# Rorisis/Co-Occ

Hardware: AMD Instinct MI355X
Metric: samples/sec (6-cam frame + sweep -> occ+render), 200x200x16 grid (higher is better)
Workload: dtype f32 (split-f16 products, fp32 accumulate)

## Files before the change

co_occ_amd/_lib.py:

```python
import ctypes
import os
import threading
import time

import torch

_HERE = os.path.dirname(os.path.abspath(__file__))
LIB_PATH = os.path.join(_HERE, "libcoocc_hip.so")

c_int, c_float, c_void_p, c_size_t, c_int64 = (ctypes.c_int, ctypes.c_float, ctypes.c_void_p,
                                               ctypes.c_size_t, ctypes.c_int64)


class ConvDesc(ctypes.Structure):
    _fields_ = [(n, c_void_p) for n in ("in_", "w", "out", "scale", "bias", "res", "gather", "out_rows", "ws")] + \
               [("ws_floats", c_int64)] + \
               [(n, c_int) for n in ("M", "Cin", "Cout", "taps", "in_stride", "out_stride", "res_stride",
                                     "B", "Xi", "Yi", "Zi", "Xo", "Yo", "Zo", "ksize", "stride", "pad",
                                     "relu", "res_mode", "splitk", "tile_hint", "kx", "ky", "kz", "px", "py", "pz",
                                     "wgroup_rows", "mfma_dtype")] + [("alpha", ctypes.c_float), ("M_dev", c_void_p), ("gather_stride", c_int), ("out16", c_void_p), ("out16_stride", c_int), ("out_h2", c_int),
                                                                   ("out_h2_twin", c_void_p), ("tile_sem", c_void_p), ("tile_sem_ints", c_int),
                                                                  ("alpha_dev", c_void_p), ("sx", c_int), ("sy", c_int), ("sz", c_int)]


# ... 40 lines not shown
    "coocc_ball_query": (I, [I, I, I, F, F, I, P, P, P, P]),
    "coocc_knn_topk": (I, [I, I, I, P, P, P, P, P]),
    "coocc_voxel_index_map": (I, [P, I, I, P, P]),
    "coocc_voxel_index_map_dev": (I, [P, I, P, I, P, P]),
    "coocc_fine_sample_voxel_dev": (I, [P, I, I, I, I, P, I, P, I, P, P, P, I, P]),
    "coocc_fine_sample_img_dev": (I, [P, I, I, I, I, P, P, L, P, P, I, I, P]),
    "coocc_fine_mlp_pre_dev": (I, [P, I, P, I, L, P, I, P, P, P, F, P, P, P, P, F, P, P, I, P, P]),
    "coocc_fine_fused": (I, [P, I, I, I, P, I, I, I, P, P, I, P, I, P, P, P, P, F, P, P, P, P, F, P, P, I, P, P, P]),
    "coocc_fine2_pack": (I, [P, P, I, P, P, P, P, P, P, P, P, P, P]),
    "coocc_fine2_h2": (I, [P, I, I, I, I, P, I, I, I, P, P, I, P, P, P, P, F, F, I, P, P, P, P]),
    "coocc_fine_sample_img_lin": (I, [P, I, I, I, I, P, P, I, I, I, P, P, I, I, P]),
    "coocc_scatter_fine_dev": (I, [P, L, P, I, I, I, P, P, I, I, I, F, P]),
    "coocc_scatter_fine_grouped": (I, [P, I, I, P, I, P, I, I, I, I, P, F, P, P]),
    "coocc_ball_query_voxels": (I, [I, F, F, I, I, I, I, P, P, P, P, P]),
    "coocc_knn_topk_voxels": (I, [I, I, I, I, I, I, P, P, P, P, I, P, P, P, P, P]),
    "coocc_knn_assign": (I, [I, I, I, I, F, P, P, P, P, P, P]),
    "coocc_knn_threshold": (I, [I, F, P, P, P, P]),
    "coocc_index_rows_i32": (I, [P, I, P, I, P, P]),
    "coocc_conv_pack_weights": (L, [P, I, I, I, I, P]),
    "coocc_conv_fwd": (I, [ctypes.POINTER(ConvDesc), P]),
    "coocc_fuser_search_ws": (Z, [ctypes.POINTER(SearchDesc)]),
    "coocc_fuser_search": (I, [ctypes.POINTER(SearchDesc), P, P]),
    "coocc_upsample_add_trilinear": (I, [P, P, I, I, I, I, I, I, I, I, P]),
    "coocc_upsample_add_trilinear_ex": (I, [P, P, I, I, I, I, I, I, I, I, P, P]),
    "coocc_occhead_mix": (I, [P, P, I, P, P, I, I, P]),
    "coocc_occhead_mix_ex": (I, [P, P, I, P, P, I, I, P, P]),
    "coocc_argmax_flags": (I, [P, I, I, I, I, P, P]),
    "coocc_fine_sample_voxel": (I, [P, I, I, I, I, P, I, I, P, P, P, I, P]),
    "coocc_fine_sample_img": (I, [P, I, I, I, I, P, P, L, P, I, I, P]),
    "coocc_fine_mlp_pre": (I, [P, I, P, I, L, P, P, P, F, P, P, P, P, F, P, P, I, P, P]),
    "coocc_fine_mlp": (I, [P, I, P, I, L, P, P, P, P, F, P, P, P, P, F, P, P, I, P, P]),
    "coocc_groupnorm_rows": (I, [P, L, I, I, I, P, P, F, I, P]),
    "coocc_groupnorm_nhwc": (I, [P, I, I, I, I, P, P, F, I, P]),
    "coocc_scatter_fine": (I, [P, L, I, I, P, P, I, I, I, F, P]),
    "coocc_camera_mats": (I, [P, P, P, P, P, P, I, I, I, I, P, P]),
    "coocc_get_geometry": (I, [P, P, P, P, I, I, I, I, P, P]),
    "coocc_bev_pool_forward": (I, [P, P, P, P, I, I, I, I, I, I, I, P, P]),
    "coocc_bev_pool_backward": (I, [P, P, P, P, I, I, I, I, I, I, I, P, P]),
    "coocc_voxel_pool_ws": (Z, [I, I]),
    "coocc_voxel_pool": (I, [P, P, I, I, I, P, I, I, I, I, P, I, P, Z, I, P]),
    "coocc_lift_splat": (I, [P, P, P, I, I, I, I, I, I, P, I, I, I, I, P, I, P, Z, I, P]),
    "coocc_lift_splat_cams": (I, [P, P, P, P, P, P, I, I, I, I, I, I, P, I, I, I, I, P, I, P, Z, I, P]),
    "coocc_lift_splat_reuse": (I, [P, P, I, I, I, I, I, I, I, I, I, P, I, P, Z, P]),
    "coocc_bev_pool_coords": (I, [P, P, I, I, I, I, I, I, P, I, P, Z, I, P]),
    "coocc_render_nearest": (I, [P, I, I, I, P, P, I, I, I, I, P, I, P, P]),
    "coocc_render_nearest_cams": (I, [P, I, I, I, P, P, P, P, P, I, I, I, I, P, I, P, P]),
    "coocc_render_activate_table": (I, [P, I, P]),
    "coocc_upsample_maps": (I, [P, I, I, I, I, P, P, P]),
    "coocc_volume_sampling": (I, [P, I, I, I, I, P, I, P, P, P, P]),
    "coocc_raw2outputs": (I, [P, P, I, I, I, F, F, P, P, P, P]),
    "coocc_render_losses": (I, [P, P, P, P, L, I, P, P, Z, P]),
    "coocc_conv_pack_weights_dev": (L, [P, I, I, I, I, P, P]),
    "coocc_wino_pack_weights_dev": (L, [P, I, I, I, I, P, P]),
    "coocc_wino_pack_weights_h2_dev": (L, [P, I, I, I, I, P, P]),
    "coocc_conv_pack_weights_h2_dev": (L, [P, I, I, I, I, P, P]),
    "coocc_wino_gradout": (I, [P, I, I, I, I, I, I, I, P, L, P]),
    "coocc_wino_ztap_table": (I, [L, I, P, P]),
    "coocc_wino_wgrad": (I, [P, P, L, I, I, I, I, P, P, I, P, L, P]),
    "coocc_rows_to_kh2": (I, [P, I, L, L, I, F, P, P, P]),
    "coocc_wino_operand_kh2": (I, [I, P, I, I, I, I, I, I, I, P, L, F, P, P]),
    "coocc_conv_wgrad_h2": (I, [P, P, L, I, I, F, P, P, I, P, L, P]),
    "coocc_wino_wgrad_h2": (I, [P, P, L, I, I, I, I, F, P, P, I, P, L, P]),
    "coocc_conv_tap_table": (I, [I, I, I, I, I, I, I, I, I, I, I, P, P]),
    "coocc_conv_epilogue_bwd": (I, [P, I, P, I, P, I, I, I, P, I, P, I, I, P, I, P, L, P]),
    "coocc_conv_epilogue_bwd_ex": (I, [P, I, P, I, P, I, I, I, P, I, P, I, I, P, I, P, L, P, P, F, P]),
    "coocc_conv_wgrad": (I, [P, I, I, P, I, P, I, I, I, I, P, I, P, L, P]),
    "coocc_conv_wgrad_h2t": (I, [P, I, I, P, I, P, I, I, I, I, P, P, I, P, L, P]),
    "coocc_gather_rows": (I, [P, I, P, I, I, P, I, P]),
    "coocc_scatter_add_rows": (I, [P, I, P, I, I, P, I, P]),
    "coocc_voxel_pool_bwd": (I, [P, I, P, I, I, I, P, I, I, I, I, P, P]),
    "coocc_lift_splat_bwd": (I, [P, I, P, P, P, I, I, I, I, I, I, P, I, I, I, I, P, P, P]),
    "coocc_render_nearest_bwd": (I, [P, I, I, I, P, P, I, I, I, I, P, P, P, P]),
    "coocc_upsample_maps_bwd": (I, [P, P, I, I, I, I, P, P]),
    "coocc_render_losses_bwd": (I, [P, P, P, P, L, I, P, P, P, P, P]),
    "coocc_upsample_trilinear_bwd": (I, [P, P, I, I, I, I, I, I, I, I, I, P]),
    "coocc_wino_input": (I, [P, I, I, I, I, I, I, I, P, L, P]),
    "coocc_wino_input_strided": (I, [P, I, I, I, I, I, I, I, P, I, L, P]),
    "coocc_sparse_tap_sum": (I, [P, P, I, I, I, I, I, P, P, I, I, P]),
    "coocc_wino_output": (I, [P, L, I, I, I, I, I, I, P, I, P, P, P, I, I, P]),
    "coocc_wino_output_ex": (I, [P, L, I, I, I, I, I, I, P, I, P, P, P, I, I, P, P]),
    "coocc_h2_overflow": (I, [I]),
    "coocc_device_fault": (I, [I]),
    "coocc_render_heads_h2": (I, [P, I, I, I, P, P, P, P, P, P, I, P, P, P, I, P]),
    "coocc_projection_params": (I, [P, P, P, P, P, P, I, P, P, P]),
    "coocc_occhead_mix_bwd": (I, [P, P, I, P, P, P, P, I, I, P]),
    "coocc_fine_sample_voxel_bwd": (I, [P, I, I, I, I, I, P, L, P, P, P]),
    "coocc_groupnorm_rows_bwd": (I, [P, P, P, L, I, I, I, P, F, I, P, P, P, P]),
    "coocc_fine_sample_img_bwd": (I, [P, I, I, I, I, I, P, P, L, P, P]),
    "coocc_groupnorm_nhwc_bwd": (I, [P, P, P, I, I, I, I, P, F, I, P, P, P, P]),
    "coocc_voxelize_ws": (Z, [I]),
    "coocc_voxelize_hard": (I, [P, I, I, P, P, I, I, P, P, P, P, P, Z, P]),
    "coocc_vfe_mean": (I, [P, P, I, I, I, I, P, I, P]),
    "coocc_sparse_index_map": (I, [P, I, I, I, I, P, P]),
    "coocc_sparse_conv_table": (I, [P, I, I, I, I, I, I, I, P, P, P]),
    "coocc_sparse_down_flags": (I, [P, I, I, I, I, I, I, I, P, P]),
    "coocc_sparse_conv_table3": (I, [P, I, I, I, I, I, I, I, I, I, I, I, I, I, P, P, P]),
    "coocc_sparse_down_flags3": (I, [P, I, I, I, I, I, I, I, I, I, I, I, I, I, I, I, I, P, P]),
    "coocc_sparse_lin_to_coors": (I, [P, I, I, I, I, P, P, P]),
    "coocc_bn_stats": (I, [P, I, I, I, P, P, P, Z, P]),
    "coocc_bn_apply": (I, [P, I, I, P, P, P, P, F, P, I, P, P]),
    "coocc_bn_backward": (I, [P, P, P, I, I, P, P, P, F, I, P, P, P, P, P, Z, P]),
    "coocc_bn_backward_sums": (I, [P, P, P, I, I, P, P, F, I, P, P, P, Z, P]),
    "coocc_bn_backward_dx": (I, [P, P, P, I, I, P, P, P, F, I, P, P, ctypes.c_double, P, P, P]),
    "coocc_predict_labels": (I, [P, L, L, L, L, I, I, I, I, I, I, I, P, P]),
    "coocc_eval_semantic": (I, [P, L, L, L, L, I, I, I, I, P, P, I, I, I, I, I, P, P]),
    "coocc_fpn_sum": (I, [P, P, I, I, I, I, I, I, P, I, P, P]),
    "coocc_zyx_to_rows": (I, [P, P, I, I, I, I, I, I, I, P]),
    "coocc_conv_tap_table3": (I, [I] * 17 + [P, P]),
    "coocc_fpn_sum_bwd": (I, [P, I, P, P, I, I, I, I, I, I, P]),
    "coocc_lidarseg_points": (I, [P, L, L, L, L, I, I, I, I, P, L, L, I, I, P, I, I, P, P, I, P, P]),
    "coocc_render_eval_stats": (L, [P, P, P, P, I, I, I, P, P, Z, P]),
    "coocc_render_panels": (I, [P, P, P, P, I, I, I, P, P]),
    "coocc_render_eval_ssim": (L, [P, P, I, I, I, ctypes.c_double, P, P, Z, P]),
    "coocc_sparse_dgrad_table3": (I, [P] + [I] * 16 + [P, P, P, P]),
    "coocc_bn_apply_ex": (I, [P, I, I, P, P, P, P, F, P, I, P, P, P]),
    "coocc_pool_labels": (I, [P, I, I, I, I, I, I, I, P, P]),
    "coocc_occ_loss_ws": (Z, [L, I]),
    "coocc_occ_loss_fwd": (I, [P, L, I, I, P, P, I, I, I, P, P, I, P, P, P, P, Z, P]),
    "coocc_occ_loss_bwd": (I, [P, L, I, I, P, P, I, P, P, P, P, I, P]),
    "coocc_depth_labels": (I, [P, I, I, I, I, F, F, I, P, P, P]),
    "coocc_depth_bce_ws": (Z, [L, I]),
    "coocc_depth_bce": (I, [P, P, I, I, I, I, F, P, P, P, Z, P]),
    "coocc_depth_bce_bwd": (I, [P, P, I, I, I, I, F, P, P, P, P]),
    "coocc_nbr_table2d": (I, [I, I, I, I, P, P]),
    "coocc_dcn_cols": (I, [P, I, P, I, I, I, I, I, I, I, I, P, P]),
    "coocc_se_gate2": (I, [P, I, I, I, I, P, P, P, P, P]),
    "coocc_cam_mean_ws": (Z, [I, I, I]),
    "coocc_cam_mean": (I, [P, I, I, I, I, P, P, Z, P]),
    "coocc_cam_bias_relu": (I, [P, I, I, I, I, P, I, P]),
    "coocc_dcn_cols_bwd": (I, [P, I, P, I, I, I, I, I, I, I, I, P, P, P, P]),
    "coocc_se_gate2_bwd_ws": (Z, [I, I, I]),
    "coocc_se_gate2_bwd": (I, [P, I, I, I, I, P, P, P, P, P, P, P, P, Z, P]),
    "coocc_cam_sum": (I, [P, I, I, I, I, P, P, Z, P]),
    "coocc_cam_add": (I, [P, P, I, I, I, P, F, P]),
    "coocc_dropout_rows": (I, [P, P, L, I, F, P, P]),
    "coocc_img_stem": (I, [P, I, I, I, P, P, P, I, I, I, P, I, P, P]),
    "coocc_maxpool2d_rows": (I, [P, I, I, I, I, I, P, I, P, P]),
    "coocc_maxpool2d_rows_bwd": (I, [P, I, P, I, I, I, I, I, P, I, P]),
    "coocc_img_stem_wgrad_ws": (Z, [I, I, I]),
    "coocc_img_stem_wgrad": (I, [P, I, I, I, P, I, I, P, P, Z, P]),
    "coocc_optim_chunk": (I, []),
    "coocc_optim_sumsq": (I, [P, P, I, P, I, P, P]),
    "coocc_optim_clip_coef": (I, [P, I, F, P, P, P, P]),
    "coocc_optim_adamw": (I, [P, P, I, P, I, P, I, P]),
    "coocc_optim_scale": (I, [P, P, I, P, I, P, P]),
    "coocc_frames_to_imgs": (I, [P, P, I, I, I, P, P, P, L, I, I, P, P, P]),
    "coocc_points_to_depth_maps": (I, [P, L, I, P, I, I, I, P, P]),
}

_lib = None


class KernelTimer:

    def __init__(self):
        self.enabled = False
        self.only = None
        self.records = []

    class _Region:
        def __init__(self, owner, tag, work):
            self.o, self.tag, self.work = owner, tag, work

        def __enter__(self):
            lvl = int(self.o.enabled)
            self.on = lvl >= 2 or (lvl == 1 and self.work > 0 and (self.o.only is None or self.tag.startswith(self.o.only)))
# ... 162 lines not shown
```

co_occ_amd/head.py:

```python
import collections
import threading

import numpy as np
import torch
from torch import nn

from . import _lib
from . import core as core_mod
from ._lib import TIMER, call, host_f32, host_i32, ptr
from .backbone import build_bn
from .core import PackCache, PackedConv, Rows, conv_rows, linear_rows, to_rows
from .registry import HEADS

_I32, _F32, _I64 = torch.int32, torch.float32, torch.int64
_FINE_LOCK = threading.Lock()
FUSED_FINE_MLP = __import__("os").environ.get("COOCC_FUSED_FINE_MLP", "1") != "0"
FINE_LINEAR_FIRST = __import__("os").environ.get("COOCC_FINE_LINEAR_FIRST", "1") != "0"
FINE_FUSED = int(__import__("os").environ.get("COOCC_FINE_FUSED", "1"))
FINE2_H2 = __import__("os").environ.get("COOCC_FINE2_H2", "1") != "0"
FINE2_IMG_INSIDE = __import__("os").environ.get("COOCC_FINE2_IMG_INSIDE", "1") == "1"
MERGED_PRED_Q = __import__("os").environ.get("COOCC_MERGED_PRED_Q", "1") != "0"
SCATTER_GROUPED = __import__("os").environ.get("COOCC_SCATTER_GROUPED", "1") != "0"


def _conv3d(conv_cfg, cin, cout, k, pad):
    cfg = dict(conv_cfg or dict(type='Conv3d'))
    t = cfg.pop("type", "Conv3d")
    if t != "Conv3d":
        raise NotImplementedError("OccHead: conv type %r" % t)
    return nn.Conv3d(cin, cout, kernel_size=k, stride=1, padding=pad, **cfg)


@HEADS.register_module()
class OccHead(nn.Module):
    def __init__(self, in_channels, out_channel, num_level=1, num_img_level=1, soft_weights=False,
                 loss_weight_cfg=None, conv_cfg=dict(type='Conv3d', bias=False),
                 norm_cfg=dict(type='GN', num_groups=32, requires_grad=True), fine_topk=20000,
                 point_cloud_range=[-51.2, -51.2, -5.0, 51.2, 51.2, 3.0], final_occ_size=[256, 256, 20],
                 empty_idx=0, visible_loss=False, balance_cls_weight=True, cascade_ratio=1,
                 sample_from_voxel=False, sample_from_img=False, train_cfg=None, test_cfg=None,
                 padding_mode='border', data_type='nus'):
        super().__init__()
        if type(in_channels) is not list:
            in_channels = [in_channels]
        if data_type != 'nus':
            raise NotImplementedError("OccHead: only the nuScenes projection branch is implemented")
        self.in_channels, self.out_channel, self.num_level = in_channels, out_channel, num_level
        self.fine_topk = fine_topk
        self.point_cloud_range = torch.tensor(np.array(point_cloud_range)).float()
        self.final_occ_size = final_occ_size
        self.cascade_ratio = cascade_ratio
        self.sample_from_voxel, self.sample_from_img = sample_from_voxel, sample_from_img
        self.padding_mode, self.data_type = padding_mode, data_type
        self.empty_idx, self.soft_weights = empty_idx, soft_weights
        self.num_img_level, self.num_point_sampling_feat = num_img_level, num_level
        lw = loss_weight_cfg or {}
        self.loss_weight_cfg = loss_weight_cfg
        self.loss_voxel_ce_weight = lw.get('loss_voxel_ce_weight', 1.0)
        self.loss_voxel_sem_scal_weight = lw.get('loss_voxel_sem_scal_weight', 1.0)
        self.loss_voxel_geo_scal_weight = lw.get('loss_voxel_geo_scal_weight', 1.0)
        self.loss_voxel_lovasz_weight = lw.get('loss_voxel_lovasz_weight', 1.0)
        from .losses import nusc_class_weights
        self.class_weights = nusc_class_weights() if balance_cls_weight else torch.ones(17) / 17
        self.visible_loss = visible_loss
        self.device_losses = False

        if cascade_ratio != 1 and (sample_from_voxel or sample_from_img):
            fine_in = 128 if sample_from_voxel else 0
            if sample_from_img:
                self.img_mlp_0 = nn.Sequential(nn.Conv2d(512, 128, 1, 1, 0), nn.GroupNorm(16, 128), nn.ReLU(inplace=True))
                self.img_mlp = nn.Sequential(nn.Linear(128, 64), nn.GroupNorm(16, 64), nn.ReLU(inplace=True))
                fine_in += 64
            self.fine_mlp = nn.Sequential(nn.Linear(fine_in, 64), nn.GroupNorm(16, 64), nn.ReLU(inplace=True),
                                          nn.Linear(64, out_channel))
        self.occ_convs = nn.ModuleList()
        for i in range(num_level):
            mid = in_channels[i] // 2
            self.occ_convs.append(nn.Sequential(_conv3d(conv_cfg, in_channels[i], mid, 3, 1), build_bn(norm_cfg, mid),
                                                nn.ReLU(inplace=True)))
        self.occ_pred_conv = nn.Sequential(_conv3d(conv_cfg, mid, mid // 2, 1, 0), build_bn(norm_cfg, mid // 2),
                                           nn.ReLU(inplace=True), _conv3d(conv_cfg, mid // 2, out_channel, 1, 0))
        if soft_weights:
            self.voxel_soft_weights = nn.Sequential(_conv3d(conv_cfg, mid, mid // 2, 1, 0), build_bn(norm_cfg, mid // 2),
                                                    nn.ReLU(inplace=True), _conv3d(conv_cfg, mid // 2, num_level, 1, 0))
        self._packs = PackCache(self)

    def _packed(self):
        def seq2(m):
            return (PackedConv(m[0].weight, bn=m[1], bias=m[0].bias, ksize=1),
                    PackedConv(m[3].weight, bias=m[3].bias, ksize=1))

        def build():
            d = dict(occ=[PackedConv(m[0].weight, bn=m[1], bias=m[0].bias, ksize=3, pad=1) for m in self.occ_convs],
                     pred=seq2(self.occ_pred_conv))
            if self.soft_weights:
                d["soft"] = seq2(self.voxel_soft_weights)
            if hasattr(self, "fine_mlp"):
                d["fine0"] = PackedConv(self.fine_mlp[0].weight, bias=self.fine_mlp[0].bias)
                d["fine3"] = PackedConv(self.fine_mlp[3].weight, bias=self.fine_mlp[3].bias)
            if hasattr(self, "img_mlp"):
                d["img0"] = PackedConv(self.img_mlp_0[0].weight.flatten(1), bias=self.img_mlp_0[0].bias)
                d["img"] = PackedConv(self.img_mlp[0].weight, bias=self.img_mlp[0].bias)
                if self.sample_from_voxel and self.fine_mlp[0].weight.shape[1] == 192:
                    d["img_nb"] = PackedConv(self.img_mlp[0].weight)
                    d["f0_vox_nb"] = PackedConv(self.fine_mlp[0].weight[:, :128].contiguous())
                    m = self.occ_pred_conv
                    if m[0].weight.shape[0] == 64 and m[0].weight.shape[1] == 128:
                        from .core import fold_bn
                        pq = PackedConv(torch.cat([m[0].weight.flatten(1), self.fine_mlp[0].weight[:, :128]], 0).contiguous())
                        sc, bi = fold_bn(m[1], m[0].bias)
                        dev = m[0].weight.device
                        pq.scale = torch.cat([sc.float().cpu(), torch.ones(64)]).to(dev).contiguous()
                        pq.bias = torch.cat([bi.float().cpu(), torch.zeros(64)]).to(dev).contiguous()
                        pq.ksize, pq.pad = 1, 0
                        d["pred_q"] = pq
            if hasattr(self, "img_mlp") and hasattr(self, "fine_mlp"):
                d["mlp_aligned"] = all(q.data_ptr() % 16 == 0 for m in (self.img_mlp, self.fine_mlp) for q in m.parameters())
                if ("img_nb" in d and self.out_channel <= 32 and self.img_mlp[1].num_groups == 16 and self.fine_mlp[1].num_groups == 16
                        and self.fine_mlp[0].weight.is_cuda):
                    dev = self.fine_mlp[0].weight.device
                    wp = torch.empty(24576, device=dev, dtype=torch.uint8)
                    cn = torch.empty(416, device=dev, dtype=_F32)
                    li, gi, l0, g0, l3 = self.img_mlp[0], self.img_mlp[1], self.fine_mlp[0], self.fine_mlp[1], self.fine_mlp[3]
                    q = lambda t: ptr(t.detach().float().contiguous())
                    call("coocc_fine2_pack", q(l0.weight), q(l3.weight), self.out_channel, q(li.bias), q(gi.weight), q(gi.bias),
                         q(l0.bias), q(g0.weight), q(g0.bias), q(l3.bias), ptr(wp), ptr(cn))
                    d["fine2"] = (wp, cn)
            return d
        return self._packs.get_modules((self,), build)

    def forward_coarse_rows(self, voxel_feats):
        from . import core
        p = self._packed()
        feats = [to_rows(f) for f in voxel_feats]
        lbr = core.Fork(2, feats[0].t.device, enable=len(feats) > 1 and not self.training)
        with lbr:
            small = [conv_rows(f, p["occ"][i], relu=True) for i, f in enumerate(feats) if i > 0]
        o0 = conv_rows(feats[0], p["occ"][0], relu=True, twin_for=((p["soft"][0],) if self.soft_weights else ()))
        occs = [o0] + small
        wlogit = None
        if self.soft_weights:
            h = conv_rows(o0, p["soft"][0], relu=True)
            wlogit = conv_rows(h, p["soft"][1], relu=False).t
        lbr.join(*[o.t for o in small])
        L = len(occs)
        levels = (_lib.c_void_p * L)(*[o.t.data_ptr() for o in occs])
        dims = host_i32([v for o in occs for v in (o.X, o.Y, o.Z)])
        out = Rows(torch.empty_like(o0.t), o0.B, o0.X, o0.Y, o0.Z, o0.C)
        tw = None
        merged = (MERGED_PRED_Q and "pred_q" in p and core.CONV_DTYPE == "f32" and self.cascade_ratio == 2 and self._fine2_h2_ok()
                  and not self.training)
        first = p["pred_q"] if merged else p["pred"][0]
        if core.wants_h2_twin(out, (first,)):
            tw = out.h2 = torch.empty_like(o0.t)
        call("coocc_occhead_mix_ex", levels, dims, L, ptr(wlogit), ptr(out.t), o0.B, o0.C, ptr(tw))
        if merged:
            hq = conv_rows(out, first, relu=64)
            h = Rows(hq.t, hq.B, hq.X, hq.Y, hq.Z, 64, 0)
            out.aux = dict(q=hq.t[:, 64:])
        else:
            h = conv_rows(out, p["pred"][0], relu=True)
        occ = conv_rows(h, p["pred"][1], relu=False)
        return out, occ

    def level_readers(self):
        return [(pc,) for pc in self._packed()["occ"]]

    def forward_coarse_voxel(self, voxel_feats):
        out, occ = self.forward_coarse_rows(voxel_feats)
        return {'out_voxel_feats': [out.as_ncdhw()], 'occ': [occ.as_ncdhw()]}

    def _image_rows(self, p, img_feats, transform, grid_rows, dev):
        f = img_feats[0]
        _, N_i, C_i, Hf, Wf = f.shape
        rows = torch.empty(N_i * Hf * Wf, C_i, device=dev, dtype=_F32)
        call("coocc_ncdhw_to_ndhwc", ptr(f[0].float().contiguous()), ptr(rows), N_i, C_i, Hf * Wf, C_i, 0)
        g = linear_rows(rows, p["img0"])
        gn = self.img_mlp_0[1]
        call("coocc_groupnorm_nhwc", ptr(g), N_i, Hf * Wf, g.shape[1], gn.num_groups, ptr(gn.weight.detach()),
             ptr(gn.bias.detach()), float(gn.eps), 1)
        params = self._projection_params(transform, grid_rows, dev)
        return g, params, (N_i, Hf, Wf)

    def fork_image_branch(self, img_feats, transform, grid_rows):
        if not (self.sample_from_img and img_feats is not None and self.cascade_ratio != 1 and not self.training and core_mod.BRANCHES):
            return None
        dev = img_feats[0].device
        br = core_mod.Fork(1, dev)
        if not br.on:
            return None
        with br:
            out = self._image_rows(self._packed(), img_feats, transform, grid_rows, dev)
        return br, out, (grid_rows.X, grid_rows.Y, grid_rows.Z)

    def _fine(self, ovf, occ, img_feats, transform, static=False, image_branch=None):
        p = self._packed()
        dev = ovf.t.device
        V, r = ovf.V, self.cascade_ratio
        assert ovf.B == 1, "OccHead fine branch: B == 1 (as the render block asserts, coocc_ray.py:571)"
        flags = torch.empty(V, device=dev, dtype=torch.uint8)
        call("coocc_argmax_flags", ptr(occ.t), V, occ.C, occ.stride, self.empty_idx, ptr(flags))
        lin = torch.empty(V, device=dev, dtype=_I32)
        cnt = torch.empty(1, device=dev, dtype=_I32)
        ws = torch.empty(V // 1024 + 2, device=dev, dtype=_I32)
        fgmap = torch.empty(V, device=dev, dtype=_I32) if SCATTER_GROUPED else None
        call("coocc_compact_flags_ex", ptr(flags), V, ptr(lin), ptr(cnt), ptr(fgmap), ptr(ws), ws.numel() * 4)
        use_img = self.sample_from_img and img_feats is not None
        if use_img and image_branch is not None:
            br, (g, params, (N_i, Hf, Wf)), grid = image_branch
            br.join(g, params)
            if grid != (ovf.X, ovf.Y, ovf.Z):
                params = self._projection_params(transform, ovf, dev)
        elif use_img:
            g, params, (N_i, Hf, Wf) = self._image_rows(p, img_feats, transform, ovf, dev)
        if static:
            return self._fine_static(p, ovf, lin, cnt, g if use_img else None, params if use_img else None, (N_i, Hf, Wf) if use_img else None,
                                     fgmap=fgmap)
        n = int(_lib.host_read(cnt)[0])
        core_mod.check_h2_overflow()
        assert n > 0, 'no foreground in coarse voxel'
        nf = n * r ** 3
        fine_xyz = torch.empty(3, nf, device=dev, dtype=_I64)
        self._note_fine(dict(xyz=fine_xyz, lin=lin, n=n, cnt=None, coarse=(ovf.X, ovf.Y, ovf.Z), map=fgmap))
        cvox = 128 if self.sample_from_voxel else 0
        fused = (FUSED_FINE_MLP and use_img and self.sample_from_voxel and ovf.C == 128 and g.shape[1] == 128
                 and self.out_channel <= 32 and self.img_mlp[1].num_groups == 16 and self.fine_mlp[1].num_groups == 16
                 and p.get("mlp_aligned", False))
        if fused and FINE_LINEAR_FIRST and "img_nb" in p:
            P = linear_rows(g, p["img_nb"])
            fused_one = self._fused_fine_ok(ovf, N_i)
            Q = ovf.aux.get("q") if (fused_one and ovf.aux and self._fine2_h2_ok() and FINE_FUSED < 2) else None
            if Q is None:
                Q = linear_rows(ovf.t, p["f0_vox_nb"], in_coff=ovf.coff, in_C=128)
            if fused_one:
                logits = torch.empty(nf, self.out_channel, device=dev, dtype=_F32)
                self._fine_fused(p, ovf, Q, P, params, (N_i, Hf, Wf), lin, n, None, fine_xyz, logits)
                return logits, fine_xyz
            vq = torch.empty(nf, 64, device=dev, dtype=_F32)
            call("coocc_fine_sample_voxel", ptr(Q), 64, ovf.X, ovf.Y, ovf.Z, ptr(lin), n, r,
                 host_i32(self.final_occ_size), ptr(fine_xyz), ptr(vq), 64)
            samp = torch.empty(nf, 64, device=dev, dtype=_F32)
            call("coocc_fine_sample_img", ptr(P), N_i, 64, Hf, Wf, ptr(params), ptr(fine_xyz), nf, ptr(samp), 64, r if r in (2, 4) else 0)
            li, gi, l0, g0, l3 = self.img_mlp[0], self.img_mlp[1], self.fine_mlp[0], self.fine_mlp[1], self.fine_mlp[3]
            logits = torch.empty(nf, self.out_channel, device=dev, dtype=_F32)
            d = lambda t: ptr(t.detach())
            with TIMER.region("k_fine_mlp<pre>", 2.0 * nf * 64 * (64 + self.out_channel)):
                call("coocc_fine_mlp_pre", ptr(samp), 64, ptr(vq), 64, nf, d(li.bias), d(gi.weight), d(gi.bias), float(gi.eps),
                     d(l0.weight), d(l0.bias), d(g0.weight), d(g0.bias), float(g0.eps), d(l3.weight), d(l3.bias),
                     self.out_channel, ptr(logits))
            return logits, fine_xyz
        cat = torch.empty(nf, cvox if fused else cvox + (64 if use_img else 0), device=dev, dtype=_F32)
        vox_feat = cat if self.sample_from_voxel else torch.empty(nf, ovf.C, device=dev, dtype=_F32)
        call("coocc_fine_sample_voxel", ptr(ovf.t), ovf.C, ovf.X, ovf.Y, ovf.Z, ptr(lin), n, r,
             host_i32(self.final_occ_size), ptr(fine_xyz), ptr(vox_feat), vox_feat.shape[1])
        if use_img:
            samp = torch.empty(nf, g.shape[1], device=dev, dtype=_F32)
            call("coocc_fine_sample_img", ptr(g), N_i, g.shape[1], Hf, Wf, ptr(params), ptr(fine_xyz), nf, ptr(samp),
                 samp.shape[1], r if r in (2, 4) else 0)
            if fused:
                li, gi, l0, g0, l3 = self.img_mlp[0], self.img_mlp[1], self.fine_mlp[0], self.fine_mlp[1], self.fine_mlp[3]
                logits = torch.empty(nf, self.out_channel, device=dev, dtype=_F32)
                d = lambda t: ptr(t.detach())
                with TIMER.region("k_fine_mlp", 2.0 * nf * 64 * (128 + 192 + self.out_channel)):
                    call("coocc_fine_mlp", ptr(samp), samp.shape[1], ptr(cat), cat.shape[1], nf,
                         d(li.weight), d(li.bias), d(gi.weight), d(gi.bias), float(gi.eps),
                         d(l0.weight), d(l0.bias), d(g0.weight), d(g0.bias), float(g0.eps),
                         d(l3.weight), d(l3.bias), self.out_channel, ptr(logits))
                return logits, fine_xyz
            linear_rows(samp, p["img"], out=cat, out_coff=cvox)
            gn = self.img_mlp[1]
            sub = cat[:, cvox:]
            call("coocc_groupnorm_rows", _lib.c_void_p(sub.data_ptr()), nf, 64, cat.shape[1], gn.num_groups,
                 ptr(gn.weight.detach()), ptr(gn.bias.detach()), float(gn.eps), 1)
        h = linear_rows(cat, p["fine0"])
        gn = self.fine_mlp[1]
        call("coocc_groupnorm_rows", ptr(h), nf, h.shape[1], h.shape[1], gn.num_groups, ptr(gn.weight.detach()),
             ptr(gn.bias.detach()), float(gn.eps), 1)
        return linear_rows(h, p["fine3"]), fine_xyz

    def _fine_static(self, p, ovf, lin, cnt, g, params, img_dims, fgmap=None):
        dev = ovf.t.device
        V, r = ovf.V, self.cascade_ratio
        ok = (FUSED_FINE_MLP and FINE_LINEAR_FIRST and g is not None and self.sample_from_voxel and ovf.C == 128 and g.shape[1] == 128
              and self.out_channel <= 32 and self.img_mlp[1].num_groups == 16 and self.fine_mlp[1].num_groups == 16
# ... 244 lines not shown
```

include/coocc_hip.h:

```cpp
#ifndef COOCC_HIP_H
#define COOCC_HIP_H

#include <stddef.h>
#include <stdint.h>

#ifdef __cplusplus
extern "C" {
#endif

#define COOCC_OK 0
#define COOCC_EINVAL (-1)
#define COOCC_EHIP (-2)
#define COOCC_ENOMEM (-3)

const char* coocc_last_error(void);
int coocc_abi_version(void);

int coocc_device_cu_count(int* n);
int coocc_stream_create_cu_mask(const uint32_t* mask_host, int nwords, void** stream_out);
int coocc_stream_destroy(void* stream);

int coocc_event_create(int flags, void** event_out);
int coocc_event_destroy(void* event);
int coocc_event_record(void* event, void* stream);
// ... 66 lines not shown
                          const int32_t* map_k, const uint32_t* offsets, int noff, const float* q, const float* key,
                          float* val, int32_t* idx, void* stream);

int coocc_knn_topk(int nq, int nk, int K, const float* q, const float* key, float* val,
                   int32_t* idx, void* stream);

int coocc_knn_assign(int nc, int K, int ns, int nq, float dist_thresh, const float* val,
                     const int32_t* nn, const int32_t* group, int32_t* winner, int32_t* out,
                     void* stream);
int coocc_knn_threshold(int nq, float dist_thresh, const float* val, const int32_t* nn,
                        int32_t* out, void* stream);
int coocc_index_rows_i32(const int32_t* base, int nbase, const int32_t* sel, int n, int32_t* rows,
                         void* stream);


int64_t coocc_conv_pack_weights(const float* w_host, int Cout, int Cin, int taps, int tap_major,
                                float* packed_host);

typedef struct coocc_conv_desc {
  const float* in;
  const float* w;
  float* out;
  const float* scale;
  const float* bias;
  const float* res;
  const int32_t* gather;
  const int32_t* out_rows;
  float* ws;
  int64_t ws_floats;
  int M, Cin, Cout, taps;
  int in_stride, out_stride, res_stride;
  int B, Xi, Yi, Zi, Xo, Yo, Zo, ksize, stride, pad;
  int relu, res_mode;
  int splitk;
  int tile_hint;
  int kx, ky, kz;
  int px, py, pz;
  int wgroup_rows;
  int mfma_dtype;
  float alpha;
  const int32_t* M_dev;
  int gather_stride;
  void* out16;
  int out16_stride;
  int out_h2;
  void* out_h2_twin;
  int32_t* tile_sem;
  int tile_sem_ints;
  const float* alpha_dev;
  int sx, sy, sz;
} coocc_conv_desc;

int coocc_conv_fwd(const coocc_conv_desc* d, void* stream);

int coocc_rows_to_bf16(const float* in, int in_stride, int64_t rows, int C, void* out_bf16, void* stream);

int coocc_rows_to_h2(const float* in, int in_stride, int64_t rows, int C, float scale, void* out_h2, void* stream);
int coocc_rows_to_h2_ex(const float* in, int in_stride, int64_t rows, int C, float scale, const float* scale_dev, void* out_h2,
                        void* stream);
int coocc_rows_to_f16(const float* in, int in_stride, int64_t rows, int C, void* out_f16, void* stream);
int coocc_rows_to_h2_gather(const float* in, int in_stride, const int32_t* row_ids, int64_t n_cap, const int32_t* n_dev,
                            int C, float scale, void* out_h2, void* stream);

int coocc_wino_input(const float* in, int in_stride, int B, int X, int Y, int Z, int C, int tile, float* V,
                     int64_t group_rows, void* stream);
int coocc_wino_input_strided(const float* in, int in_stride, int B, int X, int Y, int Z, int C, int tile, float* V,
                             int vstride, int64_t group_rows, void* stream);
int coocc_wino_input_h2(const float* in, int in_stride, int B, int X, int Y, int Z, int C, int tile, void* V,
                        int vstride, int64_t group_rows, float scale, void* stream);
int coocc_wino_input_h2_ex(const float* in, int in_stride, int B, int X, int Y, int Z, int C, int tile, void* V,
                           int vstride, int64_t group_rows, float scale, const float* scale_dev, void* stream);
int coocc_sparse_tap_sum(const float* P, const int32_t* map, int B, int X, int Y, int Z, int Cout, const float* scale,
                         float* S, int s_stride, int p_rows, void* stream);
int coocc_wino_output(const float* Mb, int64_t group_rows, int B, int X, int Y, int Z, int C, int tile, float* out,
                      int out_stride, const float* scale, const float* bias, const float* res, int res_stride,
                      int relu, void* stream);
int coocc_wino_output_ex(const float* Mb, int64_t group_rows, int B, int X, int Y, int Z, int C, int tile, float* out,
                         int out_stride, const float* scale, const float* bias, const float* res, int res_stride,
                         int relu, void* out_h2_twin, void* stream);
int coocc_render_heads_h2(const void* x_h2, int V, int Cin, int width, const void* ws0_pack, const float* bs0,
                          const float* ws1, const float* bs1, const void* const* wr_packs_host,
                          const float* const* br_host, int n_rgb_hidden, const float* wr_out, const float* br_out,
                          float* table, int activate, void* stream);
int64_t coocc_wino_pack_weights_h2_dev(const float* w, int Cout, int Cin, int tile, int dgrad, void* packed, void* stream);
int64_t coocc_conv_pack_weights_h2_dev(const float* w, int Cout, int Cin, int taps, int mode, void* packed, void* stream);
int coocc_h2_overflow(int reset);
#define COOCC_FAULT_SPARSE_ORDINAL 1
int coocc_device_fault(int reset);
int64_t coocc_wino_pack_weights_dev(const float* w, int Cout, int Cin, int tile, int dgrad, float* packed, void* stream);
int coocc_wino_gradout(const float* dy, int dy_stride, int B, int X, int Y, int Z, int C, int tile, float* dM,
                       int64_t group_rows, void* stream);
int coocc_wino_ztap_table(int64_t rows_total, int Z, int32_t* table, void* stream);
int coocc_wino_wgrad(const float* V, const float* dM, int64_t group_rows, int Z, int Cin, int Cout, int tile,
                     const int32_t* ztap_table, float* dw, int accumulate, float* ws, int64_t ws_floats,
                     void* stream);
int coocc_rows_to_kh2(const float* x, int stride, int64_t rows, int64_t rows_pad, int C, float scale, const float* scale_dev,
                      void* out_kh2, void* stream);
int coocc_wino_operand_kh2(int which, const float* x, int x_stride, int B, int X, int Y, int Z, int C, int tile, void* out_kh2,
                           int64_t group_rows, float scale, const float* scale_dev, void* stream);
int coocc_conv_wgrad_h2(const void* x_kh2, const void* dy_kh2, int64_t rows_pad, int Cin, int Cout, float alpha,
                        const float* alpha_dev, float* dw, int accumulate, float* ws, int64_t ws_floats, void* stream);
int coocc_wino_wgrad_h2(const void* V_kh2, const void* dM_kh2, int64_t group_rows, int Z, int Cin, int Cout, int tile,
                        float alpha, const float* alpha_dev, float* dw, int accumulate, float* ws, int64_t ws_floats,
                        void* stream);

int64_t coocc_conv_pack_weights_dev(const float* w, int Cout, int Cin, int taps, int mode, float* packed,
                                    void* stream);
int coocc_conv_tap_table(int B, int Xi, int Yi, int Zi, int Xo, int Yo, int Zo, int ksize, int stride, int pad,
                         int dgrad, int32_t* table, void* stream);
int coocc_conv_epilogue_bwd(const float* dout, int dout_stride, const float* out, int out_stride,
                            const float* scale, int M, int C, int relu, float* dacc, int dacc_stride,
                            float* dres, int dres_stride, int dres_accumulate, float* dbias,
                            int dbias_accumulate, float* ws, int64_t ws_floats, void* stream);
#define COOCC_AMAX_WORDS 2048
int coocc_conv_epilogue_bwd_ex(const float* dout, int dout_stride, const float* out, int out_stride,
                               const float* scale, int M, int C, int relu, float* dacc, int dacc_stride,
                               float* dres, int dres_stride, int dres_accumulate, float* dbias,
                               int dbias_accumulate, float* ws, int64_t ws_floats, uint32_t* amax_word, float* scale2,
                               float target, void* stream);
int coocc_conv_wgrad(const float* in, int in_rows, int in_stride, const float* dacc, int dacc_stride,
                     const int32_t* table, int M, int Cin, int Cout, int taps, float* dw, int accumulate,
                     float* ws, int64_t ws_floats, void* stream);
int coocc_conv_wgrad_h2t(const float* in, int in_rows, int in_stride, const float* dacc, int dacc_stride,
                         const int32_t* table, int M, int Cin, int Cout, int taps, const float* scale2,
                         float* dw, int accumulate, float* ws, int64_t ws_floats, void* stream);

int coocc_gather_rows(const float* src, int src_stride, const int32_t* idx, int n, int C, float* dst,
                      int dst_stride, void* stream);
int coocc_scatter_add_rows(const float* src, int src_stride, const int32_t* idx, int n, int C, float* dst,
                           int dst_stride, void* stream);
int coocc_voxel_pool_bwd(const float* dout, int dout_stride, const float* geom, int npts, int pts_per_batch,
                         int C, const float* lo_dx_host, int B, int X, int Y, int Z, float* dx, void* stream);
int coocc_lift_splat_bwd(const float* dout, int dout_stride, const float* depth, const float* feat_nhwc,
                         const float* geom, int N, int D, int H, int W, int C, int pts_per_batch,
                         const float* lo_dx_host, int B, int X, int Y, int Z, float* d_depth,
                         float* d_feat_nhwc, void* stream);
int coocc_render_nearest_bwd(const float* table, int X, int Y, int Z, const float* geom, const float* zvals,
                             int N, int D, int H, int W, const float* bounds_host, const float* dmaps,
                             float* dtable, void* stream);
int coocc_upsample_maps_bwd(const float* drgbs, const float* ddepths, int N, int H, int W, int scale,
                            float* dmaps, void* stream);
int coocc_render_losses_bwd(const float* rgbs, const float* depths, const float* rgb_gt, const float* depth_gt,
                            int64_t npix, int D, const float* losses_out, const float* gl, float* drgbs,
                            float* ddepths, void* stream);

int coocc_upsample_trilinear_bwd(const float* dfine, float* dcoarse, int B, int C, int Xc, int Yc, int Zc, int Xf,
                                 int Yf, int Zf, int accumulate, void* stream);

int coocc_occhead_mix_bwd(const float* const* levels_host, const int* dims_host, int L, const float* wlogit,
                          const float* dout, float* const* glevels_host, float* dwlogit, int B, int C,
                          void* stream);

int coocc_fine_sample_voxel_bwd(const float* dfeat, int dfeat_stride, int C, int X, int Y, int Z,
                                const int64_t* fine_xyz, int64_t nfine, const int* final_size_host, float* dvol,
                                void* stream);
int coocc_groupnorm_rows_bwd(const float* x, const float* y, const float* dy, int64_t n, int C, int stride, int groups,
                             const float* gamma, float eps, int relu, float* dx, float* dgamma, float* dbeta,
                             void* stream);

int coocc_fine_sample_img_bwd(const float* dfeat, int dfeat_stride, int ncam, int Ci, int Hf, int Wf,
                              const float* params, const int64_t* fine_xyz, int64_t nfine, float* dimg,
                              void* stream);
int coocc_groupnorm_nhwc_bwd(const float* x, const float* y, const float* dy, int N, int HW, int C, int groups,
                             const float* gamma, float eps, int relu, float* dx, float* dgamma, float* dbeta,
                             void* stream);

// ... 269 lines not shown
```

Before: 259.8.

## Fuse occ head pointwise tail MLPs and argmax flags into single H2 kernels

Adds two HIP kernels that run the two-layer pointwise MLP tails of the occupancy head, the soft-weight branch and the prediction branch, in one launch each. The hidden activations stay in LDS instead of going through global memory between two conv_rows calls. The prediction kernel also computes the argmax non-empty flags, so the later argmax_flags launch is skipped. This cuts launches and intermediate traffic, but it depends on strict shape and route preconditions, and the second-layer hidden values are re-split to f16 pairs inside the kernel.

```diff
diff --git a/co_occ_amd/_lib.py b/co_occ_amd/_lib.py
--- a/co_occ_amd/_lib.py
+++ b/co_occ_amd/_lib.py
@@ -146,6 +146,8 @@
     "coocc_h2_overflow": (I, [I]),
     "coocc_device_fault": (I, [I]),
     "coocc_render_heads_h2": (I, [P, I, I, I, P, P, P, P, P, P, I, P, P, P, I, P]),
+    "coocc_head_pred_h2": (I, [P, I, I, P, P, P, P, P, I, I, P, P, I, P, I, I, P, P]),
+    "coocc_head_soft_h2": (I, [P, I, I, P, P, P, P, P, I, P, P, I, P, I, P]),
     "coocc_projection_params": (I, [P, P, P, P, P, P, I, P, P, P]),
     "coocc_occhead_mix_bwd": (I, [P, P, I, P, P, P, P, I, I, P]),
     "coocc_fine_sample_voxel_bwd": (I, [P, I, I, I, I, I, P, L, P, P, P]),
diff --git a/co_occ_amd/csrc/head_tail_h2.hip b/co_occ_amd/csrc/head_tail_h2.hip
--- /dev/null
+++ b/co_occ_amd/csrc/head_tail_h2.hip
@@ -0,0 +1,321 @@
+#include <string.h>
+
+#include "conv_k.h"
+#include "h2_rows.h"
+
+typedef float f32x16 __attribute__((ext_vector_type(16)));
+typedef _Float16 f16x8 __attribute__((ext_vector_type(8)));
+
+#define HT_BM 128
+#define HT_STAGE (HT_BM * 128)
+#define HT_LST 33
+#define HT_HST 68
+#define HT_SOFT_OUT 36864
+
+struct HeadTailK {
+  const char* x; long long rowbytes;
+  int M; const int32_t* M_dev;
+  const char* w1; const float* scale1; const float* bias1;
+  float* hq; int hq_stride; int write_hidden;
+  const char* w2; const float* bias2; int nout;
+  float* out; int out_stride;
+  int empty_idx; uint8_t* flags;
+  float alpha;
+  int* h2_flag;
+  const char* zrow;
+};
+
+__device__ __forceinline__ void ht_glds16(const void* g, void* l) {
+  __builtin_amdgcn_global_load_lds((const __attribute__((address_space(1))) void*)g, (__attribute__((address_space(3))) void*)l, 16, 0, 0);
+}
+
+__device__ __forceinline__ void ht_stage_tile(const HeadTailK& p, char* As, int m0, int wave, int lane) {
+  const int srow = lane >> 3, slot = lane & 7;
+  const unsigned aq = (unsigned)((slot ^ ((4 * (wave & 1) + (srow >> 1)) & 7)) * 16);
+#pragma unroll
+  for (int c = 0; c < 4; ++c)
+#pragma unroll
+    for (int j = 0; j < 4; ++j) {
+      const int m = m0 + (j * 4 + wave) * 8 + srow;
+      const char* src = m < p.M ? p.x + ((long long)m * p.rowbytes + c * 128 + aq) : p.zrow;
+      ht_glds16(src, &As[c * HT_STAGE + (j * 4 + wave) * 8 * 128]);
+    }
+}
+
+template <int TM>
+__device__ __forceinline__ void ht_layer1(const HeadTailK& p, const char* As, int ctile, int rb0, int lane, const unsigned (&fragoff)[4],
+                                          f32x16 (&hh)[TM], f32x16 (&xx)[TM]) {
+  f16x8 breg[4][2][2];
+  const char* wcur = p.w1 + (long long)ctile * 4096 + lane * 16;
+#pragma unroll
+  for (int c = 0; c < 4; ++c)
+#pragma unroll
+    for (int s2 = 0; s2 < 2; ++s2)
+#pragma unroll
+      for (int pl = 0; pl < 2; ++pl) breg[c][s2][pl] = *(const f16x8*)(wcur + c * 16384 + (s2 * 2 + pl) * 1024);
+#pragma unroll
+  for (int i = 0; i < TM; ++i)
+#pragma unroll
+    for (int r = 0; r < 16; ++r) { hh[i][r] = 0.f; xx[i][r] = 0.f; }
+  __syncthreads();
+#pragma unroll
+  for (int c = 0; c < 4; ++c) {
+#pragma unroll
+    for (int s2 = 0; s2 < 2; ++s2) {
+      f16x8 fhi[TM], flo[TM];
+#pragma unroll
+      for (int i = 0; i < TM; ++i) {
+        fhi[i] = *(const f16x8*)&As[fragoff[2 * s2 + 0] + (c * HT_STAGE + (rb0 + i) * 4096)];
+        flo[i] = *(const f16x8*)&As[fragoff[2 * s2 + 1] + (c * HT_STAGE + (rb0 + i) * 4096)];
+      }
+#pragma unroll
+      for (int i = 0; i < TM; ++i) hh[i] = __builtin_amdgcn_mfma_f32_32x32x16_f16(breg[c][s2][0], fhi[i], hh[i], 0, 0, 0);
+#pragma unroll
+      for (int i = 0; i < TM; ++i) xx[i] = __builtin_amdgcn_mfma_f32_32x32x16_f16(breg[c][s2][1], fhi[i], xx[i], 0, 0, 0);
+#pragma unroll
+      for (int i = 0; i < TM; ++i) xx[i] = __builtin_amdgcn_mfma_f32_32x32x16_f16(breg[c][s2][0], flo[i], xx[i], 0, 0, 0);
+      __builtin_amdgcn_sched_barrier(0);
+    }
+  }
+  __syncthreads();
+}
+
+__device__ __forceinline__ f32x4 ht_epi1(const HeadTailK& p, const f32x16& hh, const f32x16& xx, int j, int n, float alpha, float lo, bool relu) {
+  f32x4 v;
+#pragma unroll
+  for (int e = 0; e < 4; ++e) v[e] = hh[4 * j + e] * alpha + xx[4 * j + e] * lo;
+  if (p.scale1) v = v * *(const f32x4*)(p.scale1 + n);
+  if (p.bias1) v = v + *(const f32x4*)(p.bias1 + n);
+  if (relu) { v[0] = fmaxf(v[0], 0.f); v[1] = fmaxf(v[1], 0.f); v[2] = fmaxf(v[2], 0.f); v[3] = fmaxf(v[3], 0.f); }
+  return v;
+}
+
+__device__ __forceinline__ void ht_store_tile(const HeadTailK& p, const float* Ls, int m0, int nrows, int tid) {
+  const int nout = p.nout;
+  for (int idx = tid; idx < nrows * nout; idx += 256) {
+    const int r = idx / nout, c = idx - r * nout;
+    p.out[(size_t)(m0 + r) * p.out_stride + c] = Ls[r * HT_LST + c];
+  }
+}
+
+__global__ __launch_bounds__(256, 2) void k_head_pred_h2(HeadTailK p) {
+  constexpr int TM = 4;
+  __shared__ __attribute__((aligned(16))) char As[4 * HT_STAGE];
+  const int m0 = blockIdx.x * HT_BM;
+  if (p.M_dev) {
+    p.M = min(p.M, *p.M_dev);
+    if (m0 >= p.M) return;
+  }
+  const int tid = threadIdx.x;
+  const int wave = __builtin_amdgcn_readfirstlane(tid >> 6), lane = tid & 63;
+  const int li = lane & 31, h = lane >> 5;
+  ht_stage_tile(p, As, m0, wave, lane);
+  unsigned fragoff[4];
+#pragma unroll
+  for (int q = 0; q < 4; ++q) {
+    const int sl = (q & 1) * 4 + 2 * (q >> 1) + h;
+    fragoff[q] = li * 128 + ((sl ^ ((li >> 1) & 7)) << 4);
+  }
+  const float alpha = p.alpha, lo = alpha * (1.f / H2_LO_SCALE);
+  const unsigned swz = (unsigned)((li >> 1) & 7);
+  {
+    f32x16 hh[TM], xx[TM];
+    ht_layer1<TM>(p, As, wave, 0, lane, fragoff, hh, xx);
+    const int nb = wave * 32 + 4 * h;
+    const bool hidden = wave < 2;
+#pragma unroll
+    for (int i = 0; i < TM; ++i) {
+      const int m = m0 + i * 32 + li;
+#pragma unroll
+      for (int j = 0; j < 4; ++j) {
+        const int n = nb + 8 * j;
+        const f32x4 v = ht_epi1(p, hh[i], xx[i], j, n, alpha, lo, hidden);
+        if (hidden) {
+          f16x4 vh, vl;
+#pragma unroll
+          for (int e = 0; e < 4; ++e) {
+            _Float16 a, b;
+            split_h2(v[e], a, b);
+            vh[e] = a; vl[e] = b;
+          }
+          const unsigned base = (unsigned)wave * HT_STAGE + (unsigned)(i * 32 + li) * 128 + 8 * h;
+          *(f16x4*)&As[base + (((unsigned)j ^ swz) << 4)] = vh;
+          *(f16x4*)&As[base + (((unsigned)(4 + j) ^ swz) << 4)] = vl;
+          if (m < p.M) h2_guard(p.h2_flag, v);
+        }
+        if (m < p.M && (!hidden || p.write_hidden)) *(f32x4*)(p.hq + (size_t)m * p.hq_stride + n) = v;
+      }
+    }
+  }
+  f16x8 b2[2][2][2];
+  {
+    const char* wcur = p.w2 + lane * 16;
+#pragma unroll
+    for (int c = 0; c < 2; ++c)
+#pragma unroll
+      for (int s2 = 0; s2 < 2; ++s2)
+#pragma unroll
+        for (int pl = 0; pl < 2; ++pl) b2[c][s2][pl] = *(const f16x8*)(wcur + c * 16384 + (s2 * 2 + pl) * 1024);
+  }
+  f32x16 hh2, xx2;
+#pragma unroll
+  for (int r = 0; r < 16; ++r) { hh2[r] = 0.f; xx2[r] = 0.f; }
+  __syncthreads();
+#pragma unroll
+  for (int c = 0; c < 2; ++c)
+#pragma unroll
+    for (int s2 = 0; s2 < 2; ++s2) {
+      const f16x8 fhi = *(const f16x8*)&As[fragoff[2 * s2 + 0] + (c * HT_STAGE + wave * 4096)];
+      const f16x8 flo = *(const f16x8*)&As[fragoff[2 * s2 + 1] + (c * HT_STAGE + wave * 4096)];
+      hh2 = __builtin_amdgcn_mfma_f32_32x32x16_f16(b2[c][s2][0], fhi, hh2, 0, 0, 0);
+      xx2 = __builtin_amdgcn_mfma_f32_32x32x16_f16(b2[c][s2][1], fhi, xx2, 0, 0, 0);
+      xx2 = __builtin_amdgcn_mfma_f32_32x32x16_f16(b2[c][s2][0], flo, xx2, 0, 0, 0);
+    }
+  float* Ls = (float*)&As[2 * HT_STAGE];
+#pragma unroll
+  for (int j = 0; j < 4; ++j)
+#pragma unroll
+    for (int e = 0; e < 4; ++e) {
+      const int n = 8 * j + 4 * h + e;
+      float v = hh2[4 * j + e] * alpha + xx2[4 * j + e] * lo;
+      if (n < p.nout) {
+        if (p.bias2) v += p.bias2[n];
+        Ls[(wave * 32 + li) * HT_LST + n] = v;
+      }
+    }
+  __syncthreads();
+  const int nrows = min(HT_BM, p.M - m0);
+  ht_store_tile(p, Ls, m0, nrows, tid);
+  if (p.flags && tid < nrows) {
+    const float* r = Ls + tid * HT_LST;
+    float best = r[0];
+    int bi = 0;
+    for (int c = 1; c < p.nout; ++c)
+      if (r[c] > best) { best = r[c]; bi = c; }
+    p.flags[m0 + tid] = bi != p.empty_idx;
+  }
+}
+
+__global__ __launch_bounds__(256, 2) void k_head_soft_h2(HeadTailK p) {
+  constexpr int TM = 2;
+  __shared__ __attribute__((aligned(16))) char As[4 * HT_STAGE];
+  const int m0 = blockIdx.x * HT_BM;
+  if (p.M_dev) {
+    p.M = min(p.M, *p.M_dev);
+    if (m0 >= p.M) return;
+  }
+  const int tid = threadIdx.x;
+  const int wave = __builtin_amdgcn_readfirstlane(tid >> 6), lane = tid & 63;
+  const int li = lane & 31, h = lane >> 5;
+  ht_stage_tile(p, As, m0, wave, lane);
+  unsigned fragoff[4];
+#pragma unroll
+  for (int q = 0; q < 4; ++q) {
+    const int sl = (q & 1) * 4 + 2 * (q >> 1) + h;
+    fragoff[q] = li * 128 + ((sl ^ ((li >> 1) & 7)) << 4);
+  }
+  float* Hs = (float*)As;
+  {
+    const int ctile = wave & 1, rb0 = 2 * (wave >> 1);
+    const float alpha = p.alpha, lo = alpha * (1.f / H2_LO_SCALE);
+    f32x16 hh[TM], xx[TM];
+    ht_layer1<TM>(p, As, ctile, rb0, lane, fragoff, hh, xx);
+    const int nb = ctile * 32 + 4 * h;
+#pragma unroll
+    for (int i = 0; i < TM; ++i) {
+      const int row = (rb0 + i) * 32 + li, m = m0 + row;
+#pragma unroll
+      for (int j = 0; j < 4; ++j) {
+        const int n = nb + 8 * j;
+        const f32x4 v = ht_epi1(p, hh[i], xx[i], j, n, alpha, lo, true);
+        *(f32x4*)&Hs[row * HT_HST + n] = v;
+        if (p.write_hidden && m < p.M) *(f32x4*)(p.hq + (size_t)m * p.hq_stride + n) = v;
+      }
+    }
+  }
+  f32x4 wb[2][4];
+#pragma unroll
+  for (int c = 0; c < 2; ++c)
+#pragma unroll
+    for (int q = 0; q < 4; ++q) wb[c][q] = *(const f32x4*)((const float*)p.w2 + c * 4096 + q * 256 + lane * 4);
+  f32x16 acc;
+#pragma unroll
+  for (int r = 0; r < 16; ++r) acc[r] = 0.f;
+  __syncthreads();
+#pragma unroll
+  for (int c = 0; c < 2; ++c)
+#pragma unroll
+    for (int q = 0; q < 4; ++q) {
+      const f32x4 a = *(const f32x4*)&Hs[(wave * 32 + li) * HT_HST + c * 32 + q * 8 + h * 4];
+#pragma unroll
+      for (int s = 0; s < 4; ++s) acc = __builtin_amdgcn_mfma_f32_32x32x2f32(a[s], wb[c][q][s], acc, 0, 0, 0);
+    }
+  float* Ls = (float*)&As[HT_SOFT_OUT];
+  if (li < p.nout) {
+    const float b = p.bias2 ? p.bias2[li] : 0.f;
+#pragma unroll
+    for (int r = 0; r < 16; ++r) {
+      float v = acc[r];
+      if (p.bias2) v += b;
+      Ls[(wave * 32 + (r & 3) + 8 * (r >> 2) + 4 * h) * HT_LST + li] = v;
+    }
+  }
+  __syncthreads();
+  ht_store_tile(p, Ls, m0, min(HT_BM, p.M - m0), tid);
+}
+
+static int ht_fill(HeadTailK& k, const char* who, const void* x_h2, int in_stride, int rows, const int32_t* rows_dev, const void* w1_pack,
+                   const float* scale1, const float* bias1, float* hidden, int hidden_stride, int hidden_min, const void* w2_pack,
+                   const float* bias2, int nout, float* out, int out_stride) {
+  COOCC_CHECK_ARG(x_h2 && w1_pack && w2_pack && out, "%s: null pointer", who);
+  COOCC_CHECK_ARG(rows >= 0 && in_stride >= 128 && in_stride % 32 == 0, "%s: 128-channel H2 rows (in_stride >= 128, a multiple of 32)", who);
+  COOCC_CHECK_ARG(nout >= 1 && nout <= 32 && out_stride >= nout, "%s: 1 .. 32 output columns, out_stride >= columns", who);
+  COOCC_CHECK_ARG(!hidden || (hidden_stride >= hidden_min && hidden_stride % 4 == 0), "%s: hidden row stride (>= %d floats, a multiple of 4)", who, hidden_min);
+  COOCC_CHECK_ARG(((uintptr_t)x_h2 & 15) == 0 && ((uintptr_t)hidden & 15) == 0 && ((uintptr_t)w1_pack & 15) == 0 && ((uintptr_t)w2_pack & 15) == 0 &&
+                      ((uintptr_t)scale1 & 15) == 0 && ((uintptr_t)bias1 & 15) == 0 && ((uintptr_t)out & 3) == 0,
+                  "%s: pointers must be 16-byte aligned", who);
+  memset(&k, 0, sizeof(k));
+  k.x = (const char*)x_h2; k.rowbytes = (long long)in_stride * 4;
+  k.M = rows; k.M_dev = rows_dev;
+  k.w1 = (const char*)w1_pack; k.scale1 = scale1; k.bias1 = bias1;
+  k.hq = hidden; k.hq_stride = hidden_stride;
+  k.w2 = (const char*)w2_pack; k.bias2 = bias2; k.nout = nout;
+  k.out = out; k.out_stride = out_stride;
+  k.alpha = 1.f;
+  const void* z = nullptr;
+  int rc = coocc_zero_row(&z);
+  if (rc != COOCC_OK) return rc;
+  k.zrow = (const char*)z;
+  return coocc_h2_flag_ptr(&k.h2_flag);
+}
+
+extern "C" int coocc_head_pred_h2(const void* x_h2, int in_stride, int rows, const int32_t* rows_dev, const void* w1_pack,
+                                  const float* scale1, const float* bias1, float* hq, int hq_stride, int write_hidden,
+                                  const void* w2_pack, const float* bias2, int ncls, float* logits, int logit_stride,
+                                  int empty_idx, uint8_t* flags, void* stream) {
+  COOCC_CHECK_ARG(hq, "head_pred_h2: null pointer");
+  HeadTailK k;
+  const int rc = ht_fill(k, "head_pred_h2", x_h2, in_stride, rows, rows_dev, w1_pack, scale1, bias1, hq, hq_stride, 128, w2_pack, bias2, ncls,
+                         logits, logit_stride);
+  if (rc != COOCC_OK) return rc;
+  if (rows == 0) return COOCC_OK;
+  k.write_hidden = write_hidden;
+  k.empty_idx = empty_idx; k.flags = flags;
+  hipLaunchKernelGGL(k_head_pred_h2, dim3(cdiv(rows, HT_BM)), dim3(256), 0, as_stream(stream), k);
+  COOCC_LAUNCH_CHECK("k_head_pred_h2");
+  return COOCC_OK;
+}
+
+extern "C" int coocc_head_soft_h2(const void* x_h2, int in_stride, int rows, const int32_t* rows_dev, const void* w1_pack,
+                                  const float* scale1, const float* bias1, float* hidden, int hidden_stride, const void* w2_pack,
+                                  const float* bias2, int L, float* wlogit, int wlogit_stride, void* stream) {
+  HeadTailK k;
+  const int rc = ht_fill(k, "head_soft_h2", x_h2, in_stride, rows, rows_dev, w1_pack, scale1, bias1, hidden, hidden_stride, 64, w2_pack, bias2, L,
+                         wlogit, wlogit_stride);
+  if (rc != COOCC_OK) return rc;
+  if (rows == 0) return COOCC_OK;
+  k.write_hidden = hidden != nullptr;
+  hipLaunchKernelGGL(k_head_soft_h2, dim3(cdiv(rows, HT_BM)), dim3(256), 0, as_stream(stream), k);
+  COOCC_LAUNCH_CHECK("k_head_soft_h2");
+  return COOCC_OK;
+}
diff --git a/co_occ_amd/head.py b/co_occ_amd/head.py
--- a/co_occ_amd/head.py
+++ b/co_occ_amd/head.py
@@ -20,6 +20,7 @@
 FINE2_H2 = __import__("os").environ.get("COOCC_FINE2_H2", "1") != "0"
 FINE2_IMG_INSIDE = __import__("os").environ.get("COOCC_FINE2_IMG_INSIDE", "1") == "1"
 MERGED_PRED_Q = __import__("os").environ.get("COOCC_MERGED_PRED_Q", "1") != "0"
+HEAD_TAIL_FUSED = True
 SCATTER_GROUPED = __import__("os").environ.get("COOCC_SCATTER_GROUPED", "1") != "0"
 
 
@@ -140,8 +141,10 @@
         occs = [o0] + small
         wlogit = None
         if self.soft_weights:
-            h = conv_rows(o0, p["soft"][0], relu=True)
-            wlogit = conv_rows(h, p["soft"][1], relu=False).t
+            wlogit = self._soft_tail(o0, p["soft"])
+            if wlogit is None:
+                h = conv_rows(o0, p["soft"][0], relu=True)
+                wlogit = conv_rows(h, p["soft"][1], relu=False).t
         lbr.join(*[o.t for o in small])
         L = len(occs)
         levels = (_lib.c_void_p * L)(*[o.t.data_ptr() for o in occs])
@@ -154,6 +157,10 @@
         if core.wants_h2_twin(out, (first,)):
             tw = out.h2 = torch.empty_like(o0.t)
         call("coocc_occhead_mix_ex", levels, dims, L, ptr(wlogit), ptr(out.t), o0.B, o0.C, ptr(tw))
+        if merged and tw is not None:
+            occ = self._pred_tail(out, first, p["pred"][1])
+            if occ is not None:
+                return out, occ
         if merged:
             hq = conv_rows(out, first, relu=64)
             h = Rows(hq.t, hq.B, hq.X, hq.Y, hq.Z, 64, 0)
@@ -162,6 +169,42 @@
             h = conv_rows(out, p["pred"][0], relu=True)
         occ = conv_rows(h, p["pred"][1], relu=False)
         return out, occ
+
+    def _tail_engine_ok(self):
+        from . import core
+        return HEAD_TAIL_FUSED and not self.training and core.CONV_ENGINE == "h2" and core.CONV_DTYPE == "f32"
+
+    def _soft_tail(self, o0, soft):
+        from . import core
+        s0, s1 = soft
+        g = (o0.B, o0.X, o0.Y, o0.Z)
+        if not (self._tail_engine_ok() and o0.C == 128 and o0.coff == 0 and s0.Cin == 128 and s0.Cout == 64 and s1.Cin == 64 and s1.Cout <= 32
+                and s0.scale is not None and s1.scale is None and s0.is_pointwise and s1.is_pointwise
+                and core.route(*g, s0) == "h2" and core.route(*g, s1) == "other"):
+            return None
+        M = o0.B * o0.V
+        wlogit = torch.empty(M, s1.Cout, device=o0.t.device, dtype=_F32)
+        with TIMER.region("k_head_soft_h2", 2.0 * M * 64 * (128 + s1.Cout)):
+            call("coocc_head_soft_h2", ptr(core.h2_rows(o0)), 128, M, None, ptr(s0.h2_pack()), ptr(s0.scale), ptr(s0.bias), None, 0,
+                 ptr(s1.w), ptr(s1.bias), s1.Cout, ptr(wlogit), s1.Cout)
+        return wlogit
+
+    def _pred_tail(self, out, pq, p1):
+        from . import core
+        g = (out.B, out.X, out.Y, out.Z)
+        if not (self._tail_engine_ok() and out.C == 128 and pq.Cout == 128 and p1.Cin == 64 and p1.Cout <= 32 and p1.scale is None
+                and p1.is_pointwise and core.route(*g, pq) == "h2" and core.route(*g, p1) == "h2"):
+            return None
+        M, dev = out.B * out.V, out.t.device
+        hq = torch.empty(M, 128, device=dev, dtype=_F32)
+        occ = Rows(torch.empty(M, p1.Cout, device=dev, dtype=_F32), out.B, out.X, out.Y, out.Z, p1.Cout)
+        flags = torch.empty(M, device=dev, dtype=torch.uint8)
+        with TIMER.region("k_head_pred_h2", 2.0 * M * (128 * 128 + 64 * p1.Cout)):
+            call("coocc_head_pred_h2", ptr(out.h2), 128, M, None, ptr(pq.h2_pack()), ptr(pq.scale), ptr(pq.bias), ptr(hq), 128, 0,
+                 ptr(p1.h2_pack()), ptr(p1.bias), p1.Cout, ptr(occ.t), p1.Cout, self.empty_idx, ptr(flags))
+        out.aux = dict(q=hq[:, 64:])
+        occ.aux = dict(flags=flags)
+        return occ
 
     def level_readers(self):
         return [(pc,) for pc in self._packed()["occ"]]
@@ -198,8 +241,10 @@
         dev = ovf.t.device
         V, r = ovf.V, self.cascade_ratio
         assert ovf.B == 1, "OccHead fine branch: B == 1 (as the render block asserts, coocc_ray.py:571)"
-        flags = torch.empty(V, device=dev, dtype=torch.uint8)
-        call("coocc_argmax_flags", ptr(occ.t), V, occ.C, occ.stride, self.empty_idx, ptr(flags))
+        flags = occ.aux.get("flags") if occ.aux else None
+        if flags is None:
+            flags = torch.empty(V, device=dev, dtype=torch.uint8)
+            call("coocc_argmax_flags", ptr(occ.t), V, occ.C, occ.stride, self.empty_idx, ptr(flags))
         lin = torch.empty(V, device=dev, dtype=_I32)
         cnt = torch.empty(1, device=dev, dtype=_I32)
         ws = torch.empty(V // 1024 + 2, device=dev, dtype=_I32)
diff --git a/include/coocc_hip.h b/include/coocc_hip.h
--- a/include/coocc_hip.h
+++ b/include/coocc_hip.h
@@ -172,6 +172,13 @@
                           const float* ws1, const float* bs1, const void* const* wr_packs_host,
                           const float* const* br_host, int n_rgb_hidden, const float* wr_out, const float* br_out,
                           float* table, int activate, void* stream);
+int coocc_head_pred_h2(const void* x_h2, int in_stride, int rows, const int32_t* rows_dev, const void* w1_pack,
+                       const float* scale1, const float* bias1, float* hq, int hq_stride, int write_hidden,
+                       const void* w2_pack, const float* bias2, int ncls, float* logits, int logit_stride,
+                       int empty_idx, uint8_t* flags, void* stream);
+int coocc_head_soft_h2(const void* x_h2, int in_stride, int rows, const int32_t* rows_dev, const void* w1_pack,
+                       const float* scale1, const float* bias1, float* hidden, int hidden_stride, const void* w2_pack,
+                       const float* bias2, int L, float* wlogit, int wlogit_stride, void* stream);
 int64_t coocc_wino_pack_weights_h2_dev(const float* w, int Cout, int Cin, int tile, int dgrad, void* packed, void* stream);
 int64_t coocc_conv_pack_weights_h2_dev(const float* w, int Cout, int Cin, int taps, int mode, void* packed, void* stream);
 int coocc_h2_overflow(int reset);
```

Result: faster. 266.8, median of 6 (+2.7%).
